# Boulder-Computer-Architecture-Lab/shrewd

Measured on AMD Instinct MI355X. Metric: fault-injection trials/sec (whole node), higher is better.
Workload: dtype int64; 1 GPU; crc32 (RV64, 64618 golden insts), 100000 single-bit x1..x31+pc trials per GPU per step; trials_per_gpu=100000, seed=0x5eed0002, structures=x1-x31,pc, burst=1, lanes_per_wave=32, parallelism=trial-sharded x1, RCCL histogram all-reduce

## Files before the change

### include/fi_engine.h

```cpp
#ifndef SHREWD_FI_ENGINE_H
#define SHREWD_FI_ENGINE_H

#ifndef __HIPCC_RTC__
#include <stddef.h>
#include <stdint.h>
#endif

#ifdef __cplusplus
extern "C" {
#endif

typedef int32_t fi_status;
#define FI_OK 0
#define FI_E_ARG -1
#define FI_E_NODEVICE -2
#define FI_E_HIP -3
#define FI_E_ELF -4
#define FI_E_STATE -5
#define FI_E_GOLDEN -6

#define FI_MASKED 0
#define FI_SDC 1
#define FI_CRASH 2
#define FI_HANG 3
// ... 70 lines not shown
    uint32_t epoch_iters;
    uint32_t lanes_per_wave;
    uint32_t resume_lanes;
    uint32_t epochs;
} fi_config;
#define FI_CFG_NO_SNAPSHOT_START 1u
#define FI_CFG_NO_EARLY_EXIT 2u
#define FI_CFG_NO_TRANSLATE 4u
#define FI_CFG_NO_EPOCHS 8u
#define FI_CFG_PACK_RUNS 16u
#define FI_CFG_FIXED_RESUME 32u
#define FI_CFG_NO_SOLO 64u
#define FI_CFG_SOLO_ALL 128u
#define FI_CFG_SIMT 256u
#define FI_CFG_NO_FORWARD 512u
#define FI_CFG_NO_SDC_EXIT 1024u
#define FI_CFG_NO_REDO 2048u
#define FI_CFG_NO_ODD_KERNEL 4096u
#define FI_CFG_JIT_NO_CACHE 8192u
#define FI_CFG_NO_HANG_PROOF 16384u
#define FI_CFG_NO_OVERFLOW 32768u
#define FI_CFG_NO_LOOP_ORDER 65536u
#define FI_CFG_NO_LOAD_AHEAD 131072u

typedef struct {
    uint64_t ninst, ncycles;
    uint32_t exit_code, pad;
    uint64_t stdout_len, stderr_len;
    uint64_t fetch_bytes, data_bytes;
    uint64_t snapshots, snapshot_interval;
    uint64_t snapshot_frames;
    uint64_t translated_blocks;
    uint64_t translated_insts;
    uint64_t translate_us;
} fi_golden_info;

typedef struct {
    uint64_t counts[FI_N_STRUCT][64][FI_N_CLASS];
    uint64_t crash_sub[16];
    uint64_t escape_sub[8];
    uint64_t trials;
    uint64_t guest_insts;
    uint64_t fetch_bytes;
    uint64_t data_bytes;
    uint64_t cow_pages;
    uint64_t device_insts;
// ... 217 lines not shown
```

### shrewd_amd/csrc/fi_engine.cpp

```cpp
#include <hip/hip_runtime.h>

#include <algorithm>
#include <atomic>
#include <chrono>
#include <condition_variable>
#include <memory>
#include <mutex>
#include <thread>
#include <cstdarg>
#include <cstdio>
#include <cstdlib>
#include <cstring>
#include <map>
#include <random>
#include <string>
#include <vector>

#include "fi_capture.h"
#include "fi_checkpoint.h"
#include "fi_debug.h"
#include "fi_exact.h"
#include "fi_golden_host.h"
#include "fi_site_draw.h"
#include "fi_tick.h"
// ... 41 lines not shown
hipError_t scan_u64(void *tmp, size_t bytes, const uint64_t *in, uint64_t *out, uint64_t n, hipStream_t st);
hipError_t sort_pairs_bytes(uint64_t n, size_t &bytes);
hipError_t launch_pack_runs(const uint64_t *keys, const uint32_t *cnt, uint64_t cap, uint32_t *wrange,
                            uint32_t *n_waves, hipStream_t st);
hipError_t launch_redo_collect(const fi_outcome *out, uint64_t n, uint32_t *idx, uint32_t *cnt,
                               unsigned long long *stats, hipStream_t st);
hipError_t launch_redo_gather(const fi_site *sites, const uint32_t *idx, uint64_t n, fi_site *rsites, uint64_t *keys,
                              uint32_t *perm, hipStream_t st);
hipError_t launch_redo_scatter(const uint32_t *idx, uint64_t n, const fi_outcome *rout, fi_outcome *out,
                               hipStream_t st);
hipError_t launch_capture_init(uint8_t *rows, uint64_t n, uint32_t stride, uint32_t cap, const uint8_t *gold,
                               uint64_t glen, hipStream_t st);
hipError_t launch_capture_finish(uint8_t *rows, uint64_t n, uint32_t stride, uint32_t cap, const fi_stream_len *lens,
                                 uint32_t err, hipStream_t st);
hipError_t launch_surv_keys(const LaneSave *save, const uint32_t *list, const uint32_t *cnt, uint64_t cap,
                            uint64_t text_lo, uint64_t *keys, uint32_t *vals, uint32_t *n_odd, uint32_t solo,
                            uint64_t golden_ninst, uint32_t nb, const LoopEst *loops, uint32_t n_loops,
                            uint64_t hang_cap, hipStream_t st);
hipError_t launch_odd_split(const uint32_t *cnt, const uint32_t *n_odd, uint32_t *split, uint32_t grid,
                            hipStream_t st);
std::string translate_blocks(const std::vector<PreInst> &pre, uint64_t text_lo, const std::vector<uint32_t> &trace,
                             const std::vector<uint64_t> &extra_pcs, std::vector<uint32_t> &leaders_out,
                             uint32_t &n_insts, bool odd_streams, std::vector<LoopEst> *loops_out = nullptr,
                             bool load_ahead = true);
std::vector<fi_issue_op> issue_ops_from_trace(const std::vector<PreInst> &pre, const std::vector<uint32_t> &trace);
std::string jit_compile(const std::string &body, const char *arch, std::vector<char> &code, bool &cached, int part,
                        bool use_cache);
bool jit_has_odd(const std::string &body);
bool jit_parallel_ok();
hipError_t sort_pairs(void *tmp, size_t bytes, const uint64_t *kin, uint64_t *kout, const uint32_t *vin,
                      uint32_t *vout, uint64_t n, int end_bit, hipStream_t st);
}

using namespace fi;

static constexpr uint32_t kDefaultLanes = 32;
static constexpr uint32_t kPreTail = 4;
static constexpr uint32_t kDefaultResumeLanes = 8;
static constexpr uint64_t kJitWindowChunk = 131072;

struct JitJob {
    std::string body, arch;
    bool odd = false;
    bool use_cache = true;
    std::vector<char> code[3];
    std::string err;
    bool cached = true;
// ... 1153 lines not shown
    if (!live_ok || g.trace.empty() || e->gold.info.ninst >= (1ULL << 29)) return FI_OK;
    std::vector<uint32_t> off, ev;
    first_access_index(g.trace, rmask, wmask, off, ev);
    HIPCHK(e->gold.d_fw_off.alloc(33));
    HIPCHK(e->gold.d_fw_ev.alloc(std::max<size_t>(ev.size(), 1)));
    HIPCHK(hipMemcpy(e->gold.d_fw_off, off.data(), 33 * 4, hipMemcpyHostToDevice));
    if (!ev.empty()) HIPCHK(hipMemcpy(e->gold.d_fw_ev, ev.data(), ev.size() * 4, hipMemcpyHostToDevice));
    e->gold.fw_off = std::move(off);
    e->gold.fw_ev = std::move(ev);
    e->gold.fw_ok = true;
    return FI_OK;
}

static fi_status golden_translate(fi_engine *e, GoldenCapture &g, bool live_ok) {
    if (e->cfg.flags & FI_CFG_NO_TRANSLATE) e->gold.tx_status = "disabled (FI_CFG_NO_TRANSLATE)";
    else if (!e->gold.pre_ok) e->gold.tx_status = "golden run rewrites its text";
    else if (!live_ok || g.trace.empty()) e->gold.tx_status = "golden trace unavailable";
    else {
        const std::vector<uint64_t> pcs;
        std::vector<uint32_t> leaders;
        std::vector<LoopEst> loops;
        uint32_t n_tx = 0;
        const bool ahead = !(e->cfg.flags & FI_CFG_NO_LOAD_AHEAD);
        std::string body = translate_blocks(g.pre, e->img.text_lo, g.trace, pcs, leaders, n_tx, true, &loops, ahead);
        if (n_tx > 24000) {
            leaders.clear();
            loops.clear();
            body = translate_blocks(g.pre, e->img.text_lo, g.trace, pcs, leaders, n_tx, false, &loops, ahead);
        }
        if (!loops.empty() && !(e->cfg.flags & FI_CFG_NO_LOOP_ORDER)) {
            HIPCHK(e->gold.d_loops.alloc(loops.size()));
            HIPCHK(hipMemcpy(e->gold.d_loops, loops.data(), loops.size() * sizeof(LoopEst), hipMemcpyHostToDevice));
            e->gold.n_loops = (uint32_t)loops.size();
        }
        e->gold.tx_body = body;
        hipDeviceProp_t prop;
        HIPCHK(hipGetDeviceProperties(&prop, e->dev));
        if (const char *dump = getenv("SHREWD_FI_DUMP_TX")) {
            if (FILE *f = fopen(dump, "w")) { fputs(body.c_str(), f); fclose(f); }
        }
        if (leaders.empty()) {
            e->gold.tx_status = "nothing to translate (no code run twice)";
        } else if (n_tx > 24000) {
            e->gold.tx_status = "translation too large";
        } else {
            auto j = std::make_shared<JitJob>();
            j->body = body;
            j->arch = prop.gcnArchName;
            j->odd = jit_has_odd(body);
            j->use_cache = !(e->cfg.flags & FI_CFG_JIT_NO_CACHE);
            for (uint32_t h : leaders) g.pre[h & 0x7FFFFFFFu].flags |= (h >> 31) ? kPreOddLeader : kPreLeader;
// ... 1366 lines not shown
    std::vector<uint32_t> t(trace, trace + n_trace), leaders;
    std::vector<LoopEst> loops;
    uint32_t n_tx = 0;
    (void)translate_blocks(p, text_lo, t, {}, leaders, n_tx, true, &loops);
    static_assert(sizeof(LoopEst) == 16, "LoopEst is 16 bytes (fi_debug.h)");
    if (out) memcpy(out, loops.data(), std::min<uint64_t>(cap, loops.size()) * sizeof(LoopEst));
    if (n) *n = loops.size();
    return FI_OK;
}

fi_status fi_debug_translate(const void *pre, uint64_t n_pre, uint64_t text_lo, const uint32_t *trace,
                             uint64_t n_trace, char *out, uint64_t cap, uint64_t *len) {
    return fi_debug_translate_flags(pre, n_pre, text_lo, trace, n_trace, 0, out, cap, len);
}

fi_status fi_debug_translate_flags(const void *pre, uint64_t n_pre, uint64_t text_lo, const uint32_t *trace,
                                   uint64_t n_trace, uint32_t flags, char *out, uint64_t cap, uint64_t *len) {
    if (!pre || !trace) return FI_E_ARG;
    std::vector<PreInst> p((const PreInst *)pre, (const PreInst *)pre + n_pre);
    std::vector<uint32_t> t(trace, trace + n_trace);
    std::vector<uint32_t> leaders;
    uint32_t n_tx = 0;
    const std::string body = translate_blocks(p, text_lo, t, {}, leaders, n_tx, true, nullptr,
                                              !(flags & FI_CFG_NO_LOAD_AHEAD));
    if (out && cap) {
        const uint64_t n = std::min<uint64_t>(cap - 1, body.size());
        memcpy(out, body.data(), n);
        out[n] = 0;
    }
    if (len) *len = body.size();
    return FI_OK;
}

fi_status fi_debug_translation(fi_engine *e, char *buf, uint64_t cap, uint64_t *len) {
    if (!e) return FI_E_ARG;
    if (buf && cap) {
        const uint64_t n = std::min<uint64_t>(cap - 1, e->gold.tx_body.size());
        memcpy(buf, e->gold.tx_body.data(), n);
        buf[n] = 0;
    }
    if (len) *len = e->gold.tx_body.size();
    return FI_OK;
}

const char *fi_debug_stat_name(uint32_t slot) {
    switch (slot) {
#define FI_STAT_NAME(name, idx, what) \
// ... 111 lines not shown
```

### shrewd_amd/csrc/fi_translate.cpp

```cpp
#include <cstdlib>
#include <cctype>
#include <cstdarg>
#include <cstdio>
#include <algorithm>
#include <cstring>
#include <map>
#include <set>
#include <unordered_map>
#include <string>
#include <vector>

#include "fi_types.h"
#include "rv64_isa.h"

namespace fi {

namespace {

struct Gen {
    const std::vector<PreInst> &pre;
    uint64_t text_lo;
    const std::set<uint32_t> &leaders;
    const std::set<uint32_t> &executed;
    std::string out;
// ... 272 lines not shown
            }
            if (top) entries.insert(header);
            headers.insert(header);
            for (uint32_t v : comp) chain[v].push_back(header);
            auto inner = removed;
            for (uint32_t v : comp) inner.insert({v, header});
            run(comp, false, inner);
        }
    }
};

struct Block {
    uint32_t h0;
    std::vector<uint32_t> insts;
    bool term;
    uint64_t opc = 0;
    std::vector<uint64_t> opcs;
};

}

std::string translate_blocks(const std::vector<PreInst> &pre, uint64_t text_lo, const std::vector<uint32_t> &trace,
                             const std::vector<uint64_t> &extra_pcs, std::vector<uint32_t> &leaders_out,
                             uint32_t &n_insts, bool odd_streams, std::vector<LoopEst> *loops_out, bool load_ahead) {
    std::set<uint32_t> executed, leaders;
    auto valid = [&](uint32_t h) { return h < pre.size() && (pre[h].flags & kPreValid); };
    std::unordered_map<uint32_t, uint32_t> runs;
    for (size_t i = 0; i < trace.size(); i++) {
        const uint32_t h = trace[i] & 0x7FFFFFFFu;
        if (valid(h)) runs[h]++;
    }
    for (size_t i = 0; i < trace.size(); i++) {
        const uint32_t h = trace[i] & 0x7FFFFFFFu;
        if (!valid(h) || runs[h] < 2) continue;
        executed.insert(h);
        const bool is_ecall = trace[i] & 0x80000000u;
        if (i == 0) leaders.insert(h);
        if (i + 1 < trace.size()) {
            const uint32_t nh = trace[i + 1] & 0x7FFFFFFFu;
            if (is_ecall || nh != h + pre[h].len / 2u) leaders.insert(nh);
        }
    }
    for (auto it = leaders.begin(); it != leaders.end();) {
        if (!executed.count(*it)) it = leaders.erase(it);
        else ++it;
    }
    for (uint32_t h : executed) {
// ... 149 lines not shown
            if (k == C_BR || k == C_JAL || k == C_JALR) { b.term = true; break; }
            pc += pre[okey(pc)].len;
        }
        blocks.push_back(b);
    }
    bool cur_odd = false;
    bool oddon = false;
    std::string SB = "S_", SD = "S_dispatch", SOB = "SO_";

    enum Edge { E_DIRECT, E_DISPATCH, E_OUT };
    auto edge = [&](uint32_t from, uint64_t pc) {
        uint32_t t;
        if (!hof(pc, t)) return E_OUT;
        return S.exits.count({from, t}) ? E_DISPATCH : E_DIRECT;
    };

    Gen g{pre, text_lo, leaders, executed, {}};
    Gen so{pre, text_lo, leaders, executed, {}};
    Gen sq{pre, text_lo, leaders, executed, {}};
    Gen sc{pre, text_lo, leaders, executed, {}};
    constexpr uint32_t kSiteCaches = 8;
    uint32_t n_sites = 0;
    std::map<uint32_t, uint32_t> ahead_sites;
    n_insts = 0;
    auto hex = [](uint64_t v) {
        char b[32];
        snprintf(b, sizeof b, "0x%llxULL", (unsigned long long)v);
        return std::string(b);
    };
    auto wgo = [&](uint32_t from, uint64_t pc) {
        const Edge k = edge(from, pc);
        uint32_t t = 0;
        hof(pc, t);
        if (k == E_DIRECT) return "goto B_" + std::to_string(t) + ";";
        return "{ spc = " + hex(pc) + (k == E_DISPATCH ? "; goto tx_dispatch; }" : "; goto tx_out; }");
    };
    const char *cold = "SCOLD";
    auto sgo = [&](uint32_t from, uint64_t pc) {
        if (oddon && (pc & 1))
            return olead.count(pc) ? "goto " + SOB + std::to_string((uint32_t)((pc - text_lo) >> 1)) + ";"
                                   : "{ spc = " + hex(pc) + "; goto S_out; }";
        if (oddon && cur_odd) return "{ spc = " + hex(pc) + "; goto " + SD + "; }";
        const Edge k = edge(from, pc);
        uint32_t t = 0;
        hof(pc, t);
        if (k == E_DIRECT) return "goto " + SB + std::to_string(t) + ";";
// ... 62 lines not shown
            case OP_addi: case OP_c_addi: case OP_c_addi4spn: case OP_c_addi16sp:
                if (A.k == AV_CNT) v = AVal{AV_CNT, 0, A.lo + imm, A.lo + imm};
                else if (A.k == AV_IND && p.rd == A.base) v = AVal{AV_IND, A.base, A.lo + imm, A.lo + imm};
                else v = av_add(A, av_const(imm, imm));
                break;
            case OP_add: case OP_c_add: v = av_add(A, B); break;
            case OP_c_mv: v = B; break;
            case OP_andi: case OP_c_andi: if (imm >= 0) v = av_const(0, imm); break;
            case OP_c_zext_b: v = av_const(0, 0xFF); break;
            case OP_c_zext_h: v = av_const(0, 0xFFFF); break;
            case OP_slli: case OP_c_slli: v = av_shl(A, imm); break;
            case OP_srli: case OP_c_srli: if (imm >= 44 && imm < 64) v = av_const(0, (int64_t)((1ULL << (64 - imm)) - 1)); break;
            case OP_sh1add: v = av_add(av_shl(A, 1), B); break;
            case OP_sh2add: v = av_add(av_shl(A, 2), B); break;
            case OP_sh3add: v = av_add(av_shl(A, 3), B); break;
            case OP_c_li: case OP_lui: v = av_const(imm, imm); break;
            default: break;
            }
            av[p.rd] = v;
        }
        return ro;
    };
    std::map<uint32_t, int> ahead_at;
    for (uint32_t H : S.headers) {
        std::vector<uint32_t> cyc;
        bool nested = false;
        for (const auto &kv : S.chain) {
            const auto pos = std::find(kv.second.begin(), kv.second.end(), H);
            if (pos == kv.second.end()) continue;
            if (pos + 1 != kv.second.end()) nested = true;
            cyc.push_back(kv.first);
        }
        if (nested || cyc.empty()) continue;
        const std::set<uint32_t> in(cyc.begin(), cyc.end());
        std::map<uint32_t, const Block *> bl;
        for (const Block &b : blocks)
            if (b.opc == 0 && in.count(b.h0)) bl[b.h0] = &b;
        if (bl.size() != in.size()) continue;
        bool ok = true;
        uint32_t writes[32] = {0};
        std::map<uint32_t, std::vector<uint32_t>> nx;
        uint32_t n_exit = 0, eblk = 0;
        bool exit_on_taken = false;
        for (const auto &kv : bl) {
            const Block &b = *kv.second;
            if (b.insts.empty()) { ok = false; break; }
            auto to = [&](uint64_t pc, bool taken) {
                uint32_t t;
                if (hof(pc, t) && in.count(t) && !S.exits.count({b.h0, t})) nx[b.h0].push_back(t);
                else { n_exit++; eblk = b.h0; exit_on_taken = taken; }
            };
            for (size_t i = 0; i < b.insts.size() && ok; i++) {
                std::string e;
                uint32_t sz;
                int sx;
                const char *cond;
                const PreInst &p = pre[b.insts[i]];
                const uint64_t pc = text_lo + 2ULL * b.insts[i];
                const Cls k = classify(p, e, sz, sx, cond);
                if (k == C_JALR || k == C_STOP || ((k == C_LOAD || k == C_STORE) && in.size() != 1)) ok = false;
                if ((k == C_ALU || k == C_JAL || k == C_LOAD) && p.rd) writes[p.rd]++;
                if (k == C_BR) { to(pc + (int64_t)p.imm, true); to(pc + p.len, false); }
                if (k == C_JAL) to(pc + (int64_t)p.imm, true);
            }
            if (ok && !b.term) to(text_lo + 2ULL * b.insts.back() + pre[b.insts.back()].len, false);
        }
        if (load_ahead && ok && in.size() == 1 && !nx[H].empty()) {
            const Block &L = *bl[H];
            const RunOff ro = runoff_walk(L, writes, 0);
            for (const ProofLoad &l : ro.loads) {
                const PreInst &p = pre[L.insts[l.pos]];
                if (!ro.stores && l.kind == 3 && p.rs1 == l.reg && p.rd && p.rd != l.reg)
                    ahead_at[L.insts[l.pos]] = (int)(int32_t)(uint32_t)l.span;
            }
        }
        if (!ok || n_exit != 1) continue;
        const Block &E = *bl[eblk];
        const PreInst &br = pre[E.insts.back()];
        uint32_t reg = 0, treg = 0;
        bool exit_when_zero = false;
        if (br.op == OP_c_beqz || br.op == OP_c_bnez) {
            reg = br.rs1;
            exit_when_zero = (br.op == OP_c_beqz) == exit_on_taken;
        } else if ((br.op == OP_beq || br.op == OP_bne) && (br.rs1 == 0) != (br.rs2 == 0)) {
            reg = br.rs1 ? br.rs1 : br.rs2;
            exit_when_zero = (br.op == OP_beq) == exit_on_taken;
        } else if ((br.op == OP_beq || br.op == OP_bne) && br.rs1 && br.rs2 && br.rs1 != br.rs2) {
            if (writes[br.rs1] == 1 && writes[br.rs2] == 0) { reg = br.rs1; treg = br.rs2; }
            else if (writes[br.rs2] == 1 && writes[br.rs1] == 0) { reg = br.rs2; treg = br.rs1; }
            exit_when_zero = (br.op == OP_beq) == exit_on_taken;
        }
        if (!reg || !exit_when_zero || writes[reg] != 1) continue;
        int step = 0;
        for (size_t i = 0; i + 1 < E.insts.size(); i++) {
            const PreInst &p = pre[E.insts[i]];
            const int a = p.imm < 0 ? -p.imm : p.imm;
            if ((p.op == OP_addi || p.op == OP_c_addi) && p.rd == reg && p.rs1 == reg && (a == 1 || a == 2 || a == 4 || a == 8))
// ... 357 lines not shown
        g.put("B_%u: { // pc 0x%llx, %u insts\n", h0, (unsigned long long)pc0, n);
        if (cur_odd)
            so_.put("%s%u: { // pc 0x%llx (odd)\n", SOB.c_str(), (uint32_t)((pc0 - text_lo) >> 1),
                    (unsigned long long)pc0);
        else
            sboth(sfmt("%s%u: { // pc 0x%llx, %u insts\n", SB.c_str(), h0, (unsigned long long)pc0, n));
        std::map<uint32_t, uint32_t> blk_ahead;
        const size_t sc_at = sc.out.size();
        if (!oddon && !cur_odd && S.chain.count(h0)) {
            uint32_t ns = n_sites;
            for (uint32_t i = 0; i < n && ns < kSiteCaches; i++) {
                std::string e;
                uint32_t sz;
                int sx;
                const char *cond;
                const Cls k = classify(pre[insts[i]], e, sz, sx, cond);
                if (k != C_LOAD && k != C_STORE) continue;
                if (k == C_LOAD && ahead_at.count(insts[i])) blk_ahead[i] = ns;
                ns++;
            }
            for (const auto &kv : blk_ahead) sc.put("  HT%u = ~0ULL;\n", kv.second);
            if (!blk_ahead.empty()) sc.put("%s%u_L: ;\n", SB.c_str(), h0);
        }
        if (!cur_odd && S.headers.count(h0)) {
            std::string rw_, rs_, rc_;
            for (uint32_t x : leaders) {
                auto it = S.chain.find(x);
                if (it == S.chain.end() || x == h0) continue;
                const auto &ch = it->second;
                const auto pos = std::find(ch.begin(), ch.end(), h0);
                if (pos == ch.end()) continue;
                const uint32_t next = (pos + 1 != ch.end()) ? *(pos + 1) : x;
                const std::string clr = S.headers.count(next) ? "" : "etgt = 0xFFFFFFFFu; ";
                const std::string sclr = S.headers.count(next) ? "" : "eon = 0; ";
                rw_ += "case " + std::to_string(x) + ": " + clr + "goto B_" + std::to_string(next) + "; ";
                rs_ += "case " + std::to_string(x) + ": " + sclr + "goto " + SB + std::to_string(next) + "; ";
                const std::string chk = (!oddon && next == x && !is_cp(x))
                    ? sfmt("if (SOVER(%uu)) { spc = %s; bst = 1u; goto S_out; } ", run_len[x], hex(g.pc_of(x)).c_str())
                    : std::string();
                rc_ += "case " + std::to_string(x) + ": " + sclr + chk + "goto " + SB + std::to_string(next) + "; ";
            }
            const char *fmt = "  if (etgt != 0xFFFFFFFFu) { if (etgt == %uu) etgt = 0xFFFFFFFFu; "
                              "else switch (etgt) { %sdefault: break; } }\n";
            const char *sfm = "  ETGT_OPAQUE(); if (__builtin_expect(eon != 0, 0)) { if (etgt == %uu) eon = 0; "
                              "else switch (etgt) { %sdefault: break; } }\n";
            g.put(fmt, h0, rw_.c_str());
            so_.put(sfm, h0, rs_.c_str());
            if (!oddon) sc.put(sfm, h0, rc_.c_str());
        }
        g.put("  if (!ult64(%s, wmin)) {\n    if (%s == pmin && ult64(pmin, owm)) TXMERGE(%s);\n"
              "    else { spc = %s; goto tx_sched; }\n  }\n", P0.c_str(), P0.c_str(), P0.c_str(), P0.c_str());
        g.put("  if (((wst + %uu > ubud) & ((wst + %uu > wbud) | (TXB(mine && rem - lst < %uu) != 0)))", n, n, n);
        if (rw) g.put(" |\n      (wwatch & (TXB(mine && (lwm & 0x%xu) != 0) != 0))", rw);
        g.put(" |\n      (wdirty & (TXB(mine && ldlo < %s && ldhi > %s) != 0))) { spc = %s; goto tx_out; }\n",
              hex(bhi).c_str(), hex(blo).c_str(), P0.c_str());
        so_.put("  if ((st + %uu > bud)", n);
        if (rw) so_.put(" | ((lwm & 0x%xu) != 0)", rw);
        so_.put(" | SDIRTY(%uu, %uu)) { spc = %s; goto S_out; }\n", (uint32_t)(blo - text_lo),
                (uint32_t)(bhi - text_lo), P0.c_str());
        if (!oddon && is_cp(h0)) sc.put("  if (SOVER(%uu)) { spc = %s; bst = 1u; goto S_out; }\n", run_len[h0], P0.c_str());
        uint32_t k_st = 0, k_xt = 0, k_fb = 0, k_db = 0;
        auto commit = [&](uint32_t st, uint32_t xt, uint32_t fb, uint32_t db) {
            if (!st) return std::string();
            std::string r = "{ const uint32_t mm_ = mine ? 0xFFFFFFFFu : 0u; lst += " + std::to_string(st) + "u & mm_; ";
            if (xt) r += "lxt += " + std::to_string(xt) + "u & mm_; ";
            if (fb) r += "lfb += " + std::to_string(fb) + "u & mm_; ";
            if (db) r += "ldb += " + std::to_string(db) + "u & mm_; ";
            return r + "wst = uni32(wst + " + std::to_string(st) + "u); } ";
        };
        auto scommit = [&](uint32_t st, uint32_t xt, uint32_t fb, uint32_t db) {
            if (!st) return std::string();
            std::string r = "SADD(" + std::to_string(st) + "u); ";
            if (xt) r += "xt += " + std::to_string(xt) + "u; ";
            if (fb) r += "fb += " + std::to_string(fb) + "u; ";
            if (db) r += "db += " + std::to_string(db) + "u; ";
            return r;
        };
        for (uint32_t i = 0; i < n; i++) {
            const PreInst &p = pre[insts[i]];
            const uint64_t pc = cur_odd ? b.opcs[i] : g.pc_of(insts[i]);
            const uint64_t ft = pc + p.len;
            const uint32_t i_inst = i;
            int sc_site = -1;
// ... 11 lines not shown
            const std::string sleave_here = "{ " + scommit(k_st, k_xt, k_fb, k_db) + "spc = " + pcb + "; goto S_out; }";
            switch (k) {
            case C_ALU: {
                const std::string v = subst(e, A, B, immb, pcb);
                if (p.rd) {
                    g.put("  TXSET(%u, %s);\n", p.rd, v.c_str());
                    sboth(sfmt("  SX(%u, %s);\n", p.rd, v.c_str()));
                }
                break;
            }
            case C_NOP:
                break;
            case C_LOAD:
                g.put("  { uint8_t *p_; const bool ok_ = tx_probe(m, %s + %s, %uu, false, p_, tx);\n", A.c_str(), immb, sz);
                g.put("    if (TXB(mine && !ok_)) %s\n", leave_here.c_str());
                {
                    const std::string pl = sfmt("  { uint8_t *p_; bool pv_; if (SCOND(!tx_probe_ld(m, %s + %s, %uu, p_, pv_))) %s\n",
                                                A.c_str(), immb, sz, sleave_here.c_str());
                    so_.out += pl;
                    if (!oddon) {
                        if (S.chain.count(h0) && n_sites < kSiteCaches) {
                            const uint32_t i = n_sites++;
                            sc_site = (int)i;
                            const std::string drop = blk_ahead.count(i_inst) ? sfmt("HT%u = ~0ULL; ", i) : std::string();
                            sc.put("  { uint8_t *p_; bool pv_; const uint64_t ea_ = %s + %s, vp_ = ea_ >> 12;\n"
                                   "    if (%s(vp_ != CV%u)) { const uint64_t e_ = tlb_find(m, vp_); if (SCOND(!e_)) %s "
                                   "SC_SET(%u, vp_, e_); %s}\n", A.c_str(), immb, cold, i, sleave_here.c_str(), i,
                                   drop.c_str());
                            if (sz > 1)
                                sc.put("    if (%s(((uint32_t)ea_ & 4095u) > %uu)) %s\n", cold, 4096u - sz, sleave_here.c_str());
                            sc.put("    p_ = SC_PTR(%u, ea_); pv_ = SC_PRIV(%u);\n", i, i);
                        } else {
                            sc.out += pl;
                        }
                    }
                }
                if (p.rd) {
                    g.put("    p_ = ok_ ? p_ : const_cast<uint8_t *>(zp);\n");
                    const std::string ld = sfmt("    uint64_t v_; if (SPRIV(pv_)) v_ = *(const g_%s *)p_; else v_ = tx_sload(p_, %uu);\n",
                                                gtype(sz), sz);
                    so_.out += ld;
                    if (!oddon && sc_site >= 0 && blk_ahead.count(i_inst)) {
                        const int stp = ahead_at[insts[i_inst]];
                        sc.put("    uint64_t v_; if (HT%d == ea_) v_ = HV%d; else v_ = *(const g_%s *)p_;\n", sc_site, sc_site,
                               gtype(sz));
                        sc.put("    if (%s(((uint32_t)ea_ & 4095u) + (uint32_t)%d > %uu)) HT%d = ~0ULL;\n"
// ... 94 lines not shown
                if (rd) sboth(sfmt("    SX(%u, %s);\n", rd, ftb.c_str()));
                sboth(sfmt("    %s spc = SUNI(t_); goto %s; }\n", scommit(k_st + 1, k_xt + xt, k_fb + p.len, k_db).c_str(),
                         SD.c_str()));
                break;
            }
            default:
                break;
            }
            k_st += 1; k_xt += xt; k_fb += p.len; k_db += (k == C_LOAD || k == C_STORE) ? sz : 0;
        }
        if (!b.term) {
            const uint64_t nxt = cur_odd ? (n ? b.opcs[n - 1] + pre[insts[n - 1]].len : pc0)
                                         : n ? g.pc_of(insts[n - 1]) + pre[insts[n - 1]].len : pc0;
            g.put("  %s %s\n", commit(k_st, k_xt, k_fb, k_db).c_str(), wgo(h0, nxt).c_str());
            sboth(sfmt("  %s %s\n", scommit(k_st, k_xt, k_fb, k_db).c_str(), sgo(h0, nxt).c_str()));
        }
        g.put("}\n");
        sboth("}\n");
        if (!blk_ahead.empty()) {
            const std::string from = sfmt("goto %s%u;", SB.c_str(), h0), to = sfmt("goto %s%u_L;", SB.c_str(), h0);
            for (size_t at = sc.out.find(from, sc_at); at != std::string::npos; at = sc.out.find(from, at + to.size()))
                sc.out.replace(at, from.size(), to);
        }
        if (cur_odd) g.out.swap(g_keep);
    }
    if (oddon) g.out.swap(g_mode);
    }
    cur_odd = false;
    leaders_out.assign(leaders.begin(), leaders.end());
    for (uint64_t pc : olead) leaders_out.push_back(0x80000000u | okey(pc));
    std::string sc_head;
    sc_head += "#undef SADD\n#undef SOVER\n#undef SDONE\n#define SADD(n_) (brem -= (n_))\n"
               "#define SOVER(n_) __builtin_expect(brem < (n_), 0)\n#define SDONE() (bud - brem)\n"
               "#define SCOLD(x) __builtin_expect(!!(x), 0)\n";
    for (uint32_t i = 0; i < kSiteCaches; i++) sc_head += sfmt("  uint64_t CV%u, CP%u; uint32_t CQ%u;\n", i, i, i);
    for (const auto &kv : ahead_sites)
        sc_head += sfmt("  %s HV%u; uint64_t HT%u;\n", kv.second == 8 ? "uint64_t" : "uint32_t", kv.first, kv.first);
    sc_head += "S_entry:\n";
    for (uint32_t i = 0; i < kSiteCaches; i++) sc_head += sfmt("  CV%u = ~0ULL; CP%u = 0; CQ%u = 0;\n", i, i, i);
    sc_head += "  goto S_dispatch;\n";
    auto hoist = [](std::string t) {
        for (const auto &[from, to] : std::vector<std::pair<std::string, std::string>>{
                 {"uint8_t *p_; ", ""}, {"bool pv_; ", ""}, {"uint64_t v_; ", ""},
                 {", vp_ = ea_ >> 12;", "; vp_ = ea_ >> 12;"}, {"const uint64_t ea_ = ", "ea_ = "},
                 {"const uint64_t e_ = ", "e_ = "}, {"const uint64_t t_ = ", "t_ = "},
                 {"const uint64_t t0_ = ", "t0_ = "}, {"const uint64_t off_ = ", "off_ = "},
                 {"const uint32_t cs_ = ", "cs_ = "}, {"const bool chg_ = ", "chg_ = "},
                 {"const bool ok_ = ", "ok_ = "}, {"const bool c_ = ", "c_ = "},
                 {"const uint64_t tk_ = ", "tk_ = "}, {"const uint32_t mm_ = ", "mm_ = "}}) {
            for (size_t at = t.find(from); at != std::string::npos; at = t.find(from, at + to.size()))
                t.replace(at, from.size(), to);
        }
        return t;
    };
    return g.out + FI_TX_SPLIT + so.out + FI_TX_SPLIT + sq.out + FI_TX_SPLIT + sc_head + hoist(sc.out);
}

}
```

### shrewd_amd/csrc/hip/fi_trial.hip

```cpp
#include "fi_rtc.h"
#include "fi_types.h"
#include "fi_device.h"
#include "rv64_isa.h"
#include "gem5_opclass_table.h"
#include "fi_softfp.h"
#include "fi_crypto.h"
#ifndef __HIPCC_RTC__
#include "fi_debug.h"
#endif

namespace fi {

template <uint32_t kNL> __device__ __forceinline__ uint32_t lane_id() {
    return kNL == 1 ? 0u : (uint32_t)threadIdx.x;
}
template <uint32_t kNL> __device__ __forceinline__ uint64_t wmin64(uint64_t v) {
    return kNL == 1 ? v : wave_min64(v);
}
template <uint32_t kNL> __device__ __forceinline__ uint64_t wsum64(uint64_t v) {
    return kNL == 1 ? v : wave_sum64(v);
}
template <uint32_t kNL> __device__ __forceinline__ uint64_t rdl64(uint64_t v, int l) {
    return kNL == 1 ? v : readlane64(v, l);
}
// ... 1294 lines not shown
}

typedef __attribute__((address_space(1))) uint8_t g_u8;
typedef __attribute__((address_space(1), aligned(1))) uint16_t g_u16;
typedef __attribute__((address_space(1), aligned(1))) uint32_t g_u32;
typedef __attribute__((address_space(1), aligned(1))) uint64_t g_u64;
#define TXB(x) (kNL == 1 ? (uint64_t)(bool)(x) : (uint64_t)__builtin_amdgcn_ballot_w64(x))
#define TXSET(r, e)                                         \
    do {                                                    \
        uint64_t t_ = (uint64_t)(e);                        \
        if (kNL > 1) __asm__ volatile("" : "+v"(t_));       \
        X##r = mine ? t_ : X##r;                            \
    } while (0)

#define SCOND(x) (x)
#define SPRIV(x) (x)
#define SUNI(x) (x)
#define SUNI32(x) (x)
#define SX(r, e) X##r = (uint64_t)(e)
#define TX_TEMPS()                                                                       \
    uint8_t *p_;                                                                         \
    bool pv_, ok_, c_, chg_;                                                             \
    uint64_t v_, ea_, vp_, e_, t_, t0_, tk_, off_;                                       \
    uint32_t cs_, mm_;                                                                   \
    (void)p_; (void)pv_; (void)ok_; (void)c_; (void)chg_; (void)v_; (void)ea_; (void)vp_; \
    (void)e_; (void)t_; (void)t0_; (void)tk_; (void)off_; (void)cs_; (void)mm_
#define ETGT_OPAQUE() __asm__ volatile("" : "+s"(eon))

struct TextRef { const PreInst *pre; uint32_t lo, hi, bytes; uint64_t clo, chi; };

__device__ __forceinline__ uint32_t tx_probe_st(const LaneMem &m, uint64_t ea, uint32_t size, uint8_t *&p,
                                               const TextRef &t) {
    const uint64_t e = tlb_find(m, ea >> 12);
    p = const_cast<uint8_t *>(page_of(e)) + (ea & 4095);
    const bool ok = (e & 1) != 0 && (uint32_t)(ea & 4095) + size <= 4096u;
    const bool code = !((ea >= t.chi) | (ea + size <= t.clo));
    return ok ? (code ? 3u : 1u) : 0u;
}
typedef __attribute__((address_space(4))) const uint32_t const_u32;

__device__ __forceinline__ bool tx_probe_ld(const LaneMem &m, uint64_t ea, uint32_t size, uint8_t *&p, bool &priv) {
    const uint64_t e = tlb_find(m, ea >> 12);
    p = const_cast<uint8_t *>(page_of(e)) + (ea & 4095);
    priv = (e & 1) != 0;
    return (e != 0) & ((uint32_t)(ea & 4095) + size <= 4096u);
}
__device__ __forceinline__ uint64_t tx_sload(const uint8_t *p, uint32_t size) {
    const uint64_t a = (uint64_t)(uintptr_t)p;
    const const_u32 *q = (const const_u32 *)(uintptr_t)(a & ~3ULL);
// ... 215 lines not shown
            }
            if (st > 0) {
                const uint64_t nx = (vpn + 1) << 12;
                if (!nx) return 0;
                i = (nx - a0 + ac - 1) / ac;
            } else {
                const uint64_t lo = vpn << 12;
                if (!lo) return 0;
                i = (a0 - lo) / ac + 1;
            }
        }
    }
    if (best_k != ~0ULL) {
        const uint64_t f = best_a;
        if (in_vma(c, m, slot, f) || (f >= m.stack_min && f < kStackBase) || (f < m.stack_min && f >= kStackBase - kMaxStack))
            return 0;
        k = best_k; fva = f;
        return 2;
    }
    return n - 1 >= (left + mm - 1) / mm ? 1 : 0;
}

#ifdef FI_TX
__device__ __noinline__ void solo_tx_clean_run(KCtx *CX, lds_u64 *R, lds_mem *mp, lds_io *io) {
    CX = (KCtx *)(uintptr_t)uni64((uint64_t)(uintptr_t)CX);
    R = (lds_u64 *)(uintptr_t)(uint32_t)__builtin_amdgcn_readfirstlane((int)(uint32_t)(uintptr_t)R);
    mp = (lds_mem *)(uintptr_t)(uint32_t)__builtin_amdgcn_readfirstlane((int)(uint32_t)(uintptr_t)mp);
    io = (lds_io *)(uintptr_t)(uint32_t)__builtin_amdgcn_readfirstlane((int)(uint32_t)(uintptr_t)io);
    LaneMem m;
    m.tv0 = mp->tv0; m.tv1 = mp->tv1; m.tv2 = mp->tv2; m.tv3 = mp->tv3;
    m.tp0 = mp->tp0; m.tp1 = mp->tp1; m.tp2 = mp->tp2; m.tp3 = mp->tp3;
    TextRef tx;
    tx.pre = CX->pre; tx.lo = (uint32_t)CX->text_lo; tx.hi = (uint32_t)(CX->text_lo >> 32);
    tx.bytes = CX->text_bytes; tx.clo = CX->code_lo; tx.chi = CX->code_hi;
    uint64_t spc = io->spc;
    const uint32_t bud = io->bud;
    uint32_t etgt = 0xFFFFFFFFu, eon = 0;
    uint32_t st = 0, xt = 0, fb = 0, db = 0;
    const uint32_t hleft = io->hleft, hok = io->hok;
    uint32_t hang = 0, bst = 0;
    uint32_t brem = bud;
#define SADD(n_) (st += (n_))
#define SOVER(n_) (st + (n_) > bud)
#define SDONE() (st)
#define TXHANG(x_, c_, m_) (hok && tx_hang_proof((x_), (c_), (m_), hleft - SDONE()))
#define TXHANGU(x_, l_, c_, m_) (hok && tx_hang_proof_u((x_), (l_), (c_), (m_), hleft - SDONE()))
#define TXLOOP(c_, m_, n_) (io->lp_cnt = (c_), io->lp_m = (m_), io->lp_n = (n_))
#define TXLD(j_, d_, o_, s_) (io->lp_ld[j_][0] = (d_), io->lp_ld[j_][1] = (uint32_t)(o_), io->lp_ld[j_][2] = (s_))
#define TXR(r) uint64_t X##r = R[r];
    TXR(1) TXR(2) TXR(3) TXR(4) TXR(5) TXR(6) TXR(7) TXR(8) TXR(9) TXR(10) TXR(11) TXR(12) TXR(13)
    TXR(14) TXR(15) TXR(16) TXR(17) TXR(18) TXR(19) TXR(20) TXR(21) TXR(22) TXR(23) TXR(24) TXR(25)
    TXR(26) TXR(27) TXR(28) TXR(29) TXR(30) TXR(31)
#undef TXR
#define SC_SET(i, vp, e) (CV##i = (vp), CP##i = ((e) & ~1ULL) - ((vp) << 12), CQ##i = (uint32_t)(e) & 1u)
#define SC_PTR(i, ea) ((uint8_t *)(uintptr_t)(CP##i + (ea)))
#define SC_PRIV(i) (CQ##i != 0u)
#undef SPRIV
#define SPRIV(x) ((x) || true)
    TX_TEMPS();
    goto S_entry;
S_out:
#define TXW(r) R[r] = X##r;
    TXW(1) TXW(2) TXW(3) TXW(4) TXW(5) TXW(6) TXW(7) TXW(8) TXW(9) TXW(10) TXW(11) TXW(12) TXW(13)
    TXW(14) TXW(15) TXW(16) TXW(17) TXW(18) TXW(19) TXW(20) TXW(21) TXW(22) TXW(23) TXW(24) TXW(25)
    TXW(26) TXW(27) TXW(28) TXW(29) TXW(30) TXW(31)
#undef TXW
#undef TXHANG
#undef TXLOOP
#undef TXLD
    io->spc = spc; io->st = SDONE(); io->xt = xt; io->fb = fb; io->db = db;
#undef SADD
#undef SOVER
#undef SDONE
#ifdef SCOLD
#undef SCOLD
#endif
#undef SPRIV
#define SPRIV(x) (x)
    io->cslo = 0xFFFFFFFFu; io->cshi = 0u; io->schg = 0u; io->hang = hang; io->bst = bst;
// ... 3232 lines not shown
```

### shrewd_amd/fi.py

```python
from __future__ import annotations

import ctypes as C
import enum
import os
from typing import Iterable, Sequence

import numpy as np

from . import build as _build

FI_OK, FI_E_ARG, FI_E_NODEVICE, FI_E_HIP, FI_E_ELF, FI_E_STATE, FI_E_GOLDEN = 0, -1, -2, -3, -4, -5, -6
CLASS_NAMES = ["masked", "sdc", "crash", "hang", "detected", "escape"]
CRASH_NAMES = {1: "panic_unknown_inst", 2: "panic_illegal_inst", 3: "panic_page_fault",
               4: "fatal_syscall_range", 5: "fatal_syscall_unimpl", 6: "fatal_proxy", 7: "abort_fd_assert",
               8: "sigtrap", 9: "fatal_stack_limit", 10: "panic_amo_line", 11: "abort_sc_line", 12: "panic_se_handler",
               13: "panic_m5op", 14: "abort_vset_sew"}
ESCAPE_NAMES = {1: "inst", 2: "syscall", 3: "csr", 4: "host", 5: "resource", 6: "undefined", 7: "timing"}
TICK_ESCAPE_NAMES = {1: "after_noncounting_tick", 2: "pc_straddle_first_fetch", 3: "pc_word_and_alignment",
                     4: "pc_aligned_mid_decode", 5: "pc_two_values", 6: "pc_on_fault_attempt",
                     7: "pc_macro_op_access", 8: "reads_curtick"}
CPU_ATOMIC, CPU_TIMING = 0, 1
TICK_MAPS = {"host": 0, "device": 1}
TICK_CONTRACTS = {"numinst": 0, "literal": 1}
HANG_NAMES = {1: "max_insts", 2: "m5_quiesce"}
# ... 84 lines not shown
                ("max_trials_per_launch", C.c_uint32), ("snapshot_interval", C.c_uint32), ("flags", C.c_uint32),
                ("epoch_iters", C.c_uint32), ("lanes_per_wave", C.c_uint32),
                ("resume_lanes", C.c_uint32), ("epochs", C.c_uint32)]


CFG_NO_SNAPSHOT_START = 1
CFG_NO_EARLY_EXIT = 2
CFG_NO_TRANSLATE = 4
CFG_NO_EPOCHS = 8
CFG_PACK_RUNS = 16
CFG_FIXED_RESUME = 32
CFG_NO_SOLO = 64
CFG_SOLO_ALL = 128
CFG_SIMT = 256
CFG_NO_FORWARD = 512
CFG_NO_SDC_EXIT = 1024
CFG_NO_REDO = 2048
CFG_NO_ODD_KERNEL = 4096
CFG_JIT_NO_CACHE = 8192
CFG_NO_HANG_PROOF = 16384
CFG_NO_OVERFLOW = 32768
CFG_NO_LOOP_ORDER = 65536
CFG_NO_LOAD_AHEAD = 131072


class GoldenInfo(C.Structure):
    _fields_ = [("ninst", C.c_uint64), ("ncycles", C.c_uint64), ("exit_code", C.c_uint32), ("pad", C.c_uint32),
                ("stdout_len", C.c_uint64), ("stderr_len", C.c_uint64), ("fetch_bytes", C.c_uint64),
                ("data_bytes", C.c_uint64), ("snapshots", C.c_uint64), ("snapshot_interval", C.c_uint64),
                ("snapshot_frames", C.c_uint64), ("translated_blocks", C.c_uint64),
                ("translated_insts", C.c_uint64), ("translate_us", C.c_uint64)]


class ExactInfo(C.Structure):
    _fields_ = [("space", C.c_uint64), ("trials", C.c_uint64), ("dead_sites", C.c_uint64), ("nbits", C.c_uint32),
                ("pad", C.c_uint32), ("classes", C.c_uint64 * N_STRUCT)]

    def as_dict(self) -> dict:
        return {"space": int(self.space), "trials": int(self.trials), "dead_sites": int(self.dead_sites),
                "nbits": int(self.nbits), "classes": {s: int(c) for s, c in enumerate(self.classes) if c}}


class _ExactMemSet(C.Structure):
    _fields_ = [("bytes", C.c_uint32), ("pad", C.c_uint32), ("positions", C.c_uint64), ("classes", C.c_uint64),
                ("dead_sites", C.c_uint64)]

# ... 939 lines not shown
```

Before: 25.84 million trials/s.

## Add loop stretch fast path for self-loops in translated solo code

For single-block self-loops whose loads are provably within the current cached page and that have no stores, the translator now emits a tight inner loop. It computes how many iterations can run without page crossing or budget overrun, then runs them with no TLB checks and no per-iteration commit bookkeeping, and adds the step counts in bulk on exit. It also keeps a walking load value one iteration ahead. This targets per-iteration overhead in hot loops such as CRC32's byte loop, at the cost of larger generated code, more live registers, and more complex JIT output.

```diff
diff --git a/include/fi_engine.h b/include/fi_engine.h
--- a/include/fi_engine.h
+++ b/include/fi_engine.h
@@ -116,6 +116,7 @@
 #define FI_CFG_NO_OVERFLOW 32768u
 #define FI_CFG_NO_LOOP_ORDER 65536u
 #define FI_CFG_NO_LOAD_AHEAD 131072u
+#define FI_CFG_NO_LOOP_STRETCH 262144u
 
 typedef struct {
     uint64_t ninst, ncycles;
diff --git a/shrewd_amd/csrc/fi_engine.cpp b/shrewd_amd/csrc/fi_engine.cpp
--- a/shrewd_amd/csrc/fi_engine.cpp
+++ b/shrewd_amd/csrc/fi_engine.cpp
@@ -87,7 +87,7 @@
 std::string translate_blocks(const std::vector<PreInst> &pre, uint64_t text_lo, const std::vector<uint32_t> &trace,
                              const std::vector<uint64_t> &extra_pcs, std::vector<uint32_t> &leaders_out,
                              uint32_t &n_insts, bool odd_streams, std::vector<LoopEst> *loops_out = nullptr,
-                             bool load_ahead = true);
+                             bool load_ahead = true, bool loop_stretch = true);
 std::vector<fi_issue_op> issue_ops_from_trace(const std::vector<PreInst> &pre, const std::vector<uint32_t> &trace);
 std::string jit_compile(const std::string &body, const char *arch, std::vector<char> &code, bool &cached, int part,
                         bool use_cache);
@@ -1287,11 +1287,12 @@
         std::vector<LoopEst> loops;
         uint32_t n_tx = 0;
         const bool ahead = !(e->cfg.flags & FI_CFG_NO_LOAD_AHEAD);
-        std::string body = translate_blocks(g.pre, e->img.text_lo, g.trace, pcs, leaders, n_tx, true, &loops, ahead);
+        const bool stretch = !(e->cfg.flags & FI_CFG_NO_LOOP_STRETCH);
+        std::string body = translate_blocks(g.pre, e->img.text_lo, g.trace, pcs, leaders, n_tx, true, &loops, ahead, stretch);
         if (n_tx > 24000) {
             leaders.clear();
             loops.clear();
-            body = translate_blocks(g.pre, e->img.text_lo, g.trace, pcs, leaders, n_tx, false, &loops, ahead);
+            body = translate_blocks(g.pre, e->img.text_lo, g.trace, pcs, leaders, n_tx, false, &loops, ahead, stretch);
         }
         if (!loops.empty() && !(e->cfg.flags & FI_CFG_NO_LOOP_ORDER)) {
             HIPCHK(e->gold.d_loops.alloc(loops.size()));
@@ -2704,7 +2705,7 @@
     std::vector<uint32_t> leaders;
     uint32_t n_tx = 0;
     const std::string body = translate_blocks(p, text_lo, t, {}, leaders, n_tx, true, nullptr,
-                                              !(flags & FI_CFG_NO_LOAD_AHEAD));
+                                              !(flags & FI_CFG_NO_LOAD_AHEAD), !(flags & FI_CFG_NO_LOOP_STRETCH));
     if (out && cap) {
         const uint64_t n = std::min<uint64_t>(cap - 1, body.size());
         memcpy(out, body.data(), n);
diff --git a/shrewd_amd/csrc/fi_translate.cpp b/shrewd_amd/csrc/fi_translate.cpp
--- a/shrewd_amd/csrc/fi_translate.cpp
+++ b/shrewd_amd/csrc/fi_translate.cpp
@@ -318,7 +318,8 @@
 
 std::string translate_blocks(const std::vector<PreInst> &pre, uint64_t text_lo, const std::vector<uint32_t> &trace,
                              const std::vector<uint64_t> &extra_pcs, std::vector<uint32_t> &leaders_out,
-                             uint32_t &n_insts, bool odd_streams, std::vector<LoopEst> *loops_out, bool load_ahead) {
+                             uint32_t &n_insts, bool odd_streams, std::vector<LoopEst> *loops_out, bool load_ahead,
+                             bool loop_stretch) {
     std::set<uint32_t> executed, leaders;
     auto valid = [&](uint32_t h) { return h < pre.size() && (pre[h].flags & kPreValid); };
     std::unordered_map<uint32_t, uint32_t> runs;
@@ -514,6 +515,7 @@
     constexpr uint32_t kSiteCaches = 8;
     uint32_t n_sites = 0;
     std::map<uint32_t, uint32_t> ahead_sites;
+    std::map<uint32_t, uint32_t> stretch_held;
     n_insts = 0;
     auto hex = [](uint64_t v) {
         char b[32];
@@ -622,6 +624,8 @@
         return ro;
     };
     std::map<uint32_t, int> ahead_at;
+    struct StretchSite { bool walk; uint32_t reg, size; int step; int64_t off, span; };
+    std::map<uint32_t, std::map<uint32_t, StretchSite>> stretch_at;
     for (uint32_t H : S.headers) {
         std::vector<uint32_t> cyc;
         bool nested = false;
@@ -665,14 +669,39 @@
             }
             if (ok && !b.term) to(text_lo + 2ULL * b.insts.back() + pre[b.insts.back()].len, false);
         }
-        if (load_ahead && ok && in.size() == 1 && !nx[H].empty()) {
+        const bool self_loop = ok && in.size() == 1 && !nx[H].empty();
+        const RunOff self_ro = self_loop && (load_ahead || loop_stretch) ? runoff_walk(*bl[H], writes, 0) : RunOff{};
+        if (load_ahead && self_loop) {
             const Block &L = *bl[H];
-            const RunOff ro = runoff_walk(L, writes, 0);
+            const RunOff &ro = self_ro;
             for (const ProofLoad &l : ro.loads) {
                 const PreInst &p = pre[L.insts[l.pos]];
                 if (!ro.stores && l.kind == 3 && p.rs1 == l.reg && p.rd && p.rd != l.reg)
                     ahead_at[L.insts[l.pos]] = (int)(int32_t)(uint32_t)l.span;
             }
+        }
+        if (loop_stretch && self_loop) {
+            const Block &L = *bl[H];
+            const PreInst &br = pre[L.insts.back()];
+            std::string e;
+            uint32_t sz;
+            int sx;
+            const char *cond;
+            const RunOff &ro = self_ro;
+            bool fit = L.term && classify(br, e, sz, sx, cond) == C_BR &&
+                       g.pc_of(L.insts.back()) + (int64_t)br.imm == g.pc_of(H) && ro.ok && !ro.stores && !ro.loads.empty();
+            std::map<uint32_t, StretchSite> sites;
+            for (const ProofLoad &l : ro.loads) {
+                const PreInst &p = pre[L.insts[l.pos]];
+                const int64_t lim = (int64_t)1 << 20;
+                if (l.kind == 3 && p.rs1 == l.reg && l.off > -lim && l.off < lim)
+                    sites[l.pos] = {true, l.reg, l.size, (int)(int32_t)(uint32_t)l.span, l.off, 0};
+                else if (l.kind == 1 && l.reg && p.rs1 && l.off > -lim && l.off < lim && (int64_t)l.span < lim)
+                    sites[l.pos] = {false, l.reg, l.size, 0, l.off, (int64_t)l.span};
+                else
+                    fit = false;
+            }
+            if (fit) stretch_at[H] = sites;
         }
         if (!ok || n_exit != 1) continue;
         const Block &E = *bl[eblk];
@@ -1076,6 +1105,23 @@
             for (const auto &kv : blk_ahead) sc.put("  HT%u = ~0ULL;\n", kv.second);
             if (!blk_ahead.empty()) sc.put("%s%u_L: ;\n", SB.c_str(), h0);
         }
+        const std::map<uint32_t, StretchSite> *stretch = nullptr;
+        std::map<uint32_t, uint32_t> st_site;
+        if (!oddon && !cur_odd && stretch_at.count(h0)) {
+            uint32_t ns = n_sites;
+            bool all = true;
+            for (uint32_t i = 0; i < n; i++) {
+                std::string e;
+                uint32_t sz;
+                int sx;
+                const char *cond;
+                if (classify(pre[insts[i]], e, sz, sx, cond) != C_LOAD) continue;
+                if (ns < kSiteCaches) st_site[i] = ns++;
+                else all = false;
+            }
+            if (all) stretch = &stretch_at[h0];
+        }
+        if (stretch) sc.put("%s%u_K: ;\n", SB.c_str(), h0);
         if (!cur_odd && S.headers.count(h0)) {
             std::string rw_, rs_, rc_;
             for (uint32_t x : leaders) {
@@ -1113,6 +1159,21 @@
         so_.put(" | SDIRTY(%uu, %uu)) { spc = %s; goto S_out; }\n", (uint32_t)(blo - text_lo),
                 (uint32_t)(bhi - text_lo), P0.c_str());
         if (!oddon && is_cp(h0)) sc.put("  if (SOVER(%uu)) { spc = %s; bst = 1u; goto S_out; }\n", run_len[h0], P0.c_str());
+        if (stretch) {
+            if (run_len[h0] > n) sc.put("  k_ = (brem - %uu) / %uu;\n", run_len[h0] - n, n);
+            else sc.put("  k_ = brem / %uu;\n", n);
+            for (const auto &kv : *stretch) {
+                const StretchSite &t = kv.second;
+                const uint32_t site = st_site[kv.first];
+                if (t.walk)
+                    sc.put("  k_ = SMINU(k_, SWALK(%u, X%u + (uint64_t)(int64_t)%lldLL, %d, %uu, %d));\n", site, t.reg,
+                           (long long)t.off, t.step, t.size, pre[insts[kv.first]].rd ? 1 : 0);
+                else
+                    sc.put("  if (!SBOUND(%u, X%u, %lldLL, %lldLL)) k_ = 0u;\n", site, t.reg, (long long)t.off,
+                           (long long)(t.off + t.span + t.size));
+            }
+            sc.put("  if (SHOT(k_ >= 2u)) goto T_%u;\n", h0);
+        }
         uint32_t k_st = 0, k_xt = 0, k_fb = 0, k_db = 0;
         auto commit = [&](uint32_t st, uint32_t xt, uint32_t fb, uint32_t db) {
             if (!st) return std::string();
@@ -1170,6 +1231,11 @@
                         if (S.chain.count(h0) && n_sites < kSiteCaches) {
                             const uint32_t i = n_sites++;
                             sc_site = (int)i;
+                            if (stretch && st_site.at(i_inst) != i) {
+                                fprintf(stderr, "fi_translate: stretch site caches out of order at pc 0x%llx\n",
+                                        (unsigned long long)pc);
+                                abort();
+                            }
                             const std::string drop = blk_ahead.count(i_inst) ? sfmt("HT%u = ~0ULL; ", i) : std::string();
                             sc.put("  { uint8_t *p_; bool pv_; const uint64_t ea_ = %s + %s, vp_ = ea_ >> 12;\n"
                                    "    if (%s(vp_ != CV%u)) { const uint64_t e_ = tlb_find(m, vp_); if (SCOND(!e_)) %s "
@@ -1310,6 +1376,54 @@
             for (size_t at = sc.out.find(from, sc_at); at != std::string::npos; at = sc.out.find(from, at + to.size()))
                 sc.out.replace(at, from.size(), to);
         }
+        if (stretch) {
+            sc.put("T_%u: { // stretch of pc 0x%llx, %u insts a pass\n  ks_ = k_;\n", h0, (unsigned long long)pc0, n);
+            for (const auto &kv : *stretch) {
+                const StretchSite &t = kv.second;
+                if (!t.walk || !pre[insts[kv.first]].rd) continue;
+                sc.put("  WV%u = *(const g_%s *)SC_PTR(%u, X%u + (uint64_t)(int64_t)%lldLL);\n"
+                       "  WP%u = SC_BASE(%u) + (uint64_t)(int64_t)%lldLL; SOPAQUE(WP%u);\n", st_site[kv.first],
+                       gtype(t.size), st_site[kv.first], t.reg, (long long)t.off, st_site[kv.first], st_site[kv.first],
+                       (long long)pre[insts[kv.first]].imm + t.step, st_site[kv.first]);
+                stretch_held[st_site[kv.first]] = t.size;
+            }
+            sc.put("T_%u_P: ;\n", h0);
+            for (uint32_t i = 0; i < n; i++) {
+                const PreInst &p = pre[insts[i]];
+                const uint64_t pc = g.pc_of(insts[i]);
+                std::string e;
+                uint32_t sz;
+                int sx;
+                const char *cond;
+                const Cls k = classify(p, e, sz, sx, cond);
+                const std::string A = Gen::R(p.rs1), B = Gen::R(p.rs2);
+                char immb[48];
+                snprintf(immb, sizeof immb, "((uint64_t)(int64_t)%dLL)", p.imm);
+                if (k == C_ALU && p.rd) sc.put("  SX(%u, %s);\n", p.rd, subst(e, A, B, immb, hex(pc)).c_str());
+                if (k == C_LOAD && p.rd) {
+                    const StretchSite &t = stretch->at(i);
+                    const uint32_t site = st_site[i];
+                    if (t.walk)
+                        sc.put("  v_ = WV%u; WV%u = *(const g_%s *)(uintptr_t)(WP%u + %s);\n", site, site, gtype(sz), site,
+                               A.c_str());
+                    else
+                        sc.put("  v_ = *(const g_%s *)SC_PTR(%u, %s + %s);\n", gtype(sz), site, A.c_str(), immb);
+                    if (sx) sc.put("  X%u = (uint64_t)(int64_t)(int%d_t)v_;\n", p.rd, sx);
+                    else sc.put("  X%u = v_;\n", p.rd);
+                }
+                if (k == C_BR) {
+                    std::string keep;
+                    for (const auto &kv : *stretch)
+                        if (kv.second.walk && pre[insts[kv.first]].rd) keep += sfmt("SKEEP(WV%u); ", st_site[kv.first]);
+                    const std::string done = keep + sfmt("SADD(%uu * d_); ", k_st) + (k_xt ? sfmt("xt += %uu * d_; ", k_xt) : "") +
+                                             (k_fb ? sfmt("fb += %uu * d_; ", k_fb) : "") +
+                                             (k_db ? sfmt("db += %uu * d_; ", k_db) : "");
+                    sc.put("  k_ -= 1u;\n  if (SCOND(!(%s))) { d_ = ks_ - k_; %s%s }\n", subst(cond, A, B, immb, hex(pc)).c_str(),
+                           done.c_str(), sgo(h0, pc + p.len).c_str());
+                    sc.put("  if (SHOT(k_ != 0u)) goto T_%u_P;\n  d_ = ks_; %sgoto %s%u_K;\n}\n", h0, done.c_str(), SB.c_str(), h0);
+                }
+            }
+        }
         if (cur_odd) g.out.swap(g_keep);
     }
     if (oddon) g.out.swap(g_mode);
@@ -1324,6 +1438,8 @@
     for (uint32_t i = 0; i < kSiteCaches; i++) sc_head += sfmt("  uint64_t CV%u, CP%u; uint32_t CQ%u;\n", i, i, i);
     for (const auto &kv : ahead_sites)
         sc_head += sfmt("  %s HV%u; uint64_t HT%u;\n", kv.second == 8 ? "uint64_t" : "uint32_t", kv.first, kv.first);
+    for (uint32_t i = 0; i < kSiteCaches; i++)
+        if (stretch_held.count(i)) sc_head += sfmt("  %s WV%u; uint64_t WP%u;\n", stretch_held[i] == 8 ? "uint64_t" : "uint32_t", i, i);
     sc_head += "S_entry:\n";
     for (uint32_t i = 0; i < kSiteCaches; i++) sc_head += sfmt("  CV%u = ~0ULL; CP%u = 0; CQ%u = 0;\n", i, i, i);
     sc_head += "  goto S_dispatch;\n";
diff --git a/shrewd_amd/csrc/hip/fi_trial.hip b/shrewd_amd/csrc/hip/fi_trial.hip
--- a/shrewd_amd/csrc/hip/fi_trial.hip
+++ b/shrewd_amd/csrc/hip/fi_trial.hip
@@ -1340,9 +1340,10 @@
     uint8_t *p_;                                                                         \
     bool pv_, ok_, c_, chg_;                                                             \
     uint64_t v_, ea_, vp_, e_, t_, t0_, tk_, off_;                                       \
-    uint32_t cs_, mm_;                                                                   \
+    uint32_t cs_, mm_, k_, ks_, d_;                                                      \
     (void)p_; (void)pv_; (void)ok_; (void)c_; (void)chg_; (void)v_; (void)ea_; (void)vp_; \
-    (void)e_; (void)t_; (void)t0_; (void)tk_; (void)off_; (void)cs_; (void)mm_
+    (void)e_; (void)t_; (void)t0_; (void)tk_; (void)off_; (void)cs_; (void)mm_; (void)k_; \
+    (void)ks_; (void)d_
 #define ETGT_OPAQUE() __asm__ volatile("" : "+s"(eon))
 
 struct TextRef { const PreInst *pre; uint32_t lo, hi, bytes; uint64_t clo, chi; };
@@ -1604,6 +1605,17 @@
 }
 
 #ifdef FI_TX
+__device__ __forceinline__ uint32_t tx_walk_room(uint64_t ea, uint64_t cv, int c, uint32_t size, bool held) {
+    const uint32_t off = (uint32_t)ea & 4095u;
+    if ((ea >> 12) != cv || off > 4096u - size) return 0u;
+    const uint32_t more = c > 0 ? (4096u - size - off) / (uint32_t)c : off / (uint32_t)-c;
+    return held ? more : more + 1u;
+}
+__device__ __forceinline__ bool tx_bound_fits(uint64_t base, uint64_t cv, int64_t lo, int64_t end) {
+    const int64_t off = (int64_t)(base & 4095u);
+    return (base >> 12) == cv && off + lo >= 0 && off + end <= 4096;
+}
+
 __device__ __noinline__ void solo_tx_clean_run(KCtx *CX, lds_u64 *R, lds_mem *mp, lds_io *io) {
     CX = (KCtx *)(uintptr_t)uni64((uint64_t)(uintptr_t)CX);
     R = (lds_u64 *)(uintptr_t)(uint32_t)__builtin_amdgcn_readfirstlane((int)(uint32_t)(uintptr_t)R);
@@ -1637,6 +1649,13 @@
 #define SC_SET(i, vp, e) (CV##i = (vp), CP##i = ((e) & ~1ULL) - ((vp) << 12), CQ##i = (uint32_t)(e) & 1u)
 #define SC_PTR(i, ea) ((uint8_t *)(uintptr_t)(CP##i + (ea)))
 #define SC_PRIV(i) (CQ##i != 0u)
+#define SWALK(i, ea, c, sz, held) tx_walk_room((ea), CV##i, (c), (sz), (held) != 0)
+#define SBOUND(i, base, lo, end) tx_bound_fits((base), CV##i, (lo), (end))
+#define SC_BASE(i) (CP##i)
+#define SOPAQUE(x) __asm__ volatile("" : "+s"(x))
+#define SKEEP(x) __asm__ volatile("" : : "v"(x))
+#define SMINU(a, b) ((a) < (b) ? (a) : (b))
+#define SHOT(x) __builtin_expect(!!(x), 1)
 #undef SPRIV
 #define SPRIV(x) ((x) || true)
     TX_TEMPS();
diff --git a/shrewd_amd/fi.py b/shrewd_amd/fi.py
--- a/shrewd_amd/fi.py
+++ b/shrewd_amd/fi.py
@@ -130,6 +130,7 @@
 CFG_NO_OVERFLOW = 32768
 CFG_NO_LOOP_ORDER = 65536
 CFG_NO_LOAD_AHEAD = 131072
+CFG_NO_LOOP_STRETCH = 262144
 
 
 class GoldenInfo(C.Structure):
```

New measurement: 27.61 million trials/s (median of 6 runs). 6.9% higher.
